# azedarach/matrix-factorization-case-studies

Hardware: AMD Instinct MI355X
Metric: AA SPG outer iterations/sec (synthetic 100000x4096, k=32) (higher is better)
Workload: dtype f32; 1 GPU; AA n=100000 p=4096 k=32, X row-sharded over 1 GPU(s), init=random, delta=0, dictionary spg max_iterations=1, default weights QP; parallelism=rows/1

## Files before the change

matrix-factorization-case-studies_amd/csrc/aa_internal.h:

```cpp
#pragma once
#include <hip/hip_runtime.h>

#include <cstdarg>
#include <cstdio>
#include <cstdlib>
#include <cstring>
#include <string>
#include <vector>

#include "../../include/aa_hip.h"

namespace aa {

void set_error(const char *fmt, ...);

#define AA_CHECK_HIP(expr)                                                              \
    do {                                                                                \
        hipError_t e__ = (expr);                                                        \
        if (e__ != hipSuccess) {                                                        \
            aa::set_error("%s:%d: %s -> %s", __FILE__, __LINE__, #expr,                 \
                          hipGetErrorString(e__));                                      \
            return AA_ERR_HIP;                                                          \
        }                                                                               \
    } while (0)
// ... 165 lines not shown
    hipStream_t stream = nullptr;
    hipStream_t stream2 = nullptr;
    hipStream_t stream3 = nullptr;
    hipEvent_t evFork = nullptr, evJoin = nullptr;
    DevBuf slotCosts, slotCounters, slotStates, slotCost0;
    int slots_R = 0, slots_k = 0, slots_stride = 0, slots_max_outer = 0;
    bool slots_aa = false, slots_started = false;
    unsigned slots_cold = 0;
    unsigned slots_cold_cols = 0xffffffffu;
    DevBuf slotSaveP, slotSaveGr;
    DevBuf slotSnapP;
    aa_iter_params slots_ip;
    aa_spg_params slots_sp, slots_scale_sp;
    aa_gpnh_params slots_gp;
    aa_qp_params slots_qp;
    DevBuf qpLive;
    long qp_live_cap = 0;
    int qp_live_epoch = 0;
    char pass_names[2][48] = {{0}, {0}};
    char qp_names[192] = {0};
    char spg_path[512] = {0};
    bool spg_path_full = false;
    bool qp_tail_pending = false;
    hipEvent_t evFork2 = nullptr, evJoin2 = nullptr;
    bool qp_perm_ready = false;
    long qp_perm_n = 0;
    bool side_pending = false;
    DevBuf tmpTall2, redPartial2, redOut2, proj2, projList2, projSegCnt2;
    int projPassHint2[4] = {0, 0, 0, 0};
    bool projWarm2[4] = {false, false, false, false};
    bool time_gemm = false;
    std::vector<hipEvent_t> gemmEvents[2];
    const int *qp_tail_rows = nullptr;
    const unsigned int *qp_tail_count = nullptr;
    Comm *comm = nullptr;
    P2P *p2p = nullptr;
    int rank = 0, world = 1;
    bool force_comm = false;
    struct RidePost {
        bool on = false;
        int kind = 0, mode = 0, NV = 0, slot = 0, gated = 0, stage_after = -1;
        unsigned max_mask = 0u;
        aa_spg_params sp;
        double *red = nullptr;
        ProjState *ps = nullptr;
        double *gather = nullptr;
        long count = 0;
    };
    RidePost ride, ride_grad;
    double *ride_dst = nullptr;
    long ride_count = 0;
    double *ride_gather_next = nullptr;
    bool weights_follow = false;
    bool ride_grad_next = false;

    int form = AA_FORM_DATA;
    long n = 0, n_pad = 0, p = 0, p_pad = 0, n_global = 0, row_offset = 0;
    DevBuf X;
    bool have_data = false;
    double trace = 0.0;
    bool have_trace = false;

    int k = 0, KP = 0;
    bool have_state = false, grams_valid = false, gpnh_valid = false;
    std::vector<double> alpha;
    std::vector<double> ZtZ, CKCt, CKZ;
    bool dict_inputs_overridden = false;

    DevBuf Ct, Zt, Dt, Gr, Gn, gk, gn, H, tmpTall;
    DevBuf P, Q, ZtX, Pw, Qw;
    DevBuf wideScratch;
    DevBuf partial;
    DevBuf groupFlags;
    DevBuf slabMode;
    DevBuf rlPartial;
    DevBuf redPartial;
    DevBuf gramOut;
    DevBuf gramState;
    DevBuf costDev;
    DevBuf costSlot;
    bool host_grams_valid = false;
    DevBuf redOut;
    DevBuf redGather;
    DevBuf listGather;
    DevBuf scalars;
    DevBuf proj;
    DevBuf projList, projSegCnt;
    DevBuf Mdev, alphaDev;
    DevBuf iterState, snapC, snapZ, snapAlpha;
    DevBuf qpIters;
    DevBuf qpPerm;
    DevBuf feat, featNorm;
    long feat_p = 0, feat_ld = 0;
    KernelSpec kernel;
    DevBuf crossX, crossNorm, crossV, rowNorm, xformCost;
    long cross_s = 0, cross_s_pad = 0;
    int cross_k = 0;
    KernelSpec cross;
    DevBuf scoreScratch;
    DevBuf fsScratch;
    int fs_k = 0;
    size_t fs_off_col = 0, fs_off_st = 0, fs_off_alive = 0;
    bool qp_iters_valid = false;
    bool linear_kernel = false;
    DevBuf qpStats;
    void *hostPinned = nullptr;
    size_t hostPinnedBytes = 0;

    long nslab = 0, rows_per_slab = 0;
    int tallBlocks = 0;
    int projPassHint[4] = {0, 0, 0, 0};
    bool projWarm[4] = {false, false, false, false};
    long projCounts[4] = {0, 0, 0, 0};
    bool projListShort[4] = {false, false, false, false};
    bool x_feasible = false;
    bool products_valid = false;
    bool ckz_valid = false;
};

void spg_name(Ctx *c, const char *fmt, ...) __attribute__((format(printf, 2, 3)));
#define SPG_NAME(...) spg_name(c, __VA_ARGS__)

inline bool has_stored_data(const Ctx *c) { return c->have_data && !c->kernel.kind && c->form == AA_FORM_DATA; }

int launch_reduce_rows(Ctx *c, const double *A_tall, double *out_wide, void *outT,
                       bool main_only = false, DevBuf *flag_buf = nullptr);
#define AA_SLAB_MODE_BYTES 256
#define REDUCE_SPARSE_DEFAULT_DEN(dtype) ((dtype) == AA_F32 ? 4 : 2)
int launch_reduce_rows_finish(Ctx *c, double *out_wide, void *outT, int extra_slabs);
int launch_reduce_rows_fixup(Ctx *c, const unsigned int *count_dev, const int *rows_dev,
                             const double *zslot, const double *Ztall);
int launch_row_local(Ctx *c, const void *B_wideT, double *out_tall);
int launch_stream_probe(Ctx *c, int variant);

int tall_setup(Ctx *c);
int launch_proj(Ctx *c, const double *x, const double *g, double a_const, int a_slot, int mode,
                const aa_spg_params *sp = nullptr, int stage_after = -1);
enum { PROJ_FEAS = 0, PROJ_ALPHA = 1, PROJ_DIR = 2, PROJ_RES = 3 };
int launch_grad(Ctx *c, const double *Graw, const double *H, double *gout, double scale,
                const double *d_for_dot , int dot_slot, double *xupd = nullptr,
                const aa_spg_params *sp = nullptr, int stage_after = -1,
                const aa_spg_params *setup_sp = nullptr , double setup_fnorm = 0.0);
int launch_tall_axpy_lambda(Ctx *c, double *x, const double *d);
int launch_group_flags(Ctx *c, const double *A_tall, unsigned char *flags, unsigned int *counters);
int launch_tall_dot_scaled(Ctx *c, const double *x, const double *H, const double *alpha_dev,
                           int slot);
int launch_gram_tall(Ctx *c, const double *A, const double *B, double *out_dev, bool local_only = false);
int launch_ride_post(Ctx *c, Ctx::RidePost *rp, const double *gather);
#define AA_WIDE_TAIL(KP) ((size_t)(KP) * (KP) + (size_t)64 * 4 * (KP))
int launch_gram_wide(Ctx *c, const double *A, const double *B, double *out_dev);
int launch_scale_gram(Ctx *c, double *dst, const double *src);
int launch_aa_cost(Ctx *c, double *out_dev, int *slot_counter_dev = nullptr, const LoopJudge *judge = nullptr);
int launch_set_scalars(Ctx *c, double trace, double fnorm);
int launch_wide_axpy_lambda(Ctx *c, double *P, const double *Q, void *PT);
int launch_wide_to_T(Ctx *c, const double *src, void *dstT);
int launch_transpose_wide_to_tall(Ctx *c, const double *wide, double *tall);
int launch_transpose_tall_to_wide(Ctx *c, const double *tall, double *wide, void *wideT);
int launch_scalar_stage(Ctx *c, int stage, const aa_spg_params *sp, int it);
int launch_linesearch_fused(Ctx *c, const aa_spg_params *sp, double *cost_out, int *cost_slot);
int launch_dict_setup(Ctx *c, const aa_spg_params *sp, double fnorm, unsigned slotmask = 0xffffffffu);
int launch_iter_judge(Ctx *c, const LoopJudge &jd, const double *costs, bool judged, bool wide_dict);
int launch_cost_carry(Ctx *c, double *costs, int *slot, double cost0);
int launch_scale_factors(Ctx *c, const aa_spg_params *sp, double delta_box, const LoopJudge &jd,
                         const double *costs, const int *slot);
int launch_col_has_nan(Ctx *c, const void *raw_dev, int host_dtype, long ld, long n_total, long p_full,
                       const double *w_dev , unsigned char *flags_dev);
int launch_gather_weight(Ctx *c, const void *raw_dev, int host_dtype, long ld, long row0, long n,
                         const int *idx_dev, long p_valid, const double *w_dev);
int launch_data_to_double(Ctx *c, double *out_dev);
#define AA_MOMENT_MAX_SLABS 2048
long moment_slab_rows(long n, long p_pad, long *nslab_out);
int launch_col_moments(Ctx *c, double *partial_dev , double *mean_dev ,
                       double *var_dev );
int launch_affine_rows(Ctx *c, const void *owner_X, long row0, const double *shift_dev ,
                       const double *scale_dev );
#define AA_MAX_COEF_ROWS 16
int launch_col_weighted_sums(Ctx *c, int G, const double *At_dev , const int *grp_dev ,
                             const double *centre_dev ,
                             double *partial_dev , double *out_dev );
int launch_model_rows(Ctx *c, const void *owner_X, long row0, const int *grp_dev, const double *shift_dev,
                      const double *icpt_dev, const double *slope_dev, const double *t_dev, const double *scale_dev,
                      void *dst = nullptr );
int launch_gather_rows(Ctx *c, const void *owner_X, int owner_dtype, long owner_ld, const long *idx_dev,
                       void *dst = nullptr );
int launch_features_from_data(Ctx *c, const void *owner_X, int owner_dtype, long owner_ld, long n, long p, double *F,
                              long ldf);
int launch_gpnh_solve(Ctx *c, double lambda, int *ok_dev);
int launch_gpnh_solve_slots(Ctx *c, double lambda);
int launch_gpnh_cost_slots(Ctx *c, double lambda, unsigned mask, int what, const JudgeRule &rule, bool form_gram);
int launch_gpnh_snap_slots(Ctx *c);
int launch_aa_cost_slots(Ctx *c, int what, const JudgeRule &rule);
int launch_aa_snap_slots(Ctx *c);
int launch_qp_slots_aa(Ctx *c, const aa_qp_params *p);
int launch_qp_slots(Ctx *c, int R, int k, const double *gram_dev, const aa_qp_params *p);
bool gpnh_cost_can_gram(const Ctx *c);
int launch_gpnh_cost(Ctx *c, double lambda, double *out_dev, int *slot_counter, bool from_wide = false,
                     bool gram_w = false, const LoopJudge *judge = nullptr);
enum { ST_INIT_F = 0, ST_ALPHA = 1, ST_LINESEARCH = 2, ST_BB = 3, ST_CONV = 4 };
int launch_row_sqnorm_sum(Ctx *c, double *trace_out_host);
int launch_distance_column(Ctx *c, long j_local, int owner_has_row, const double *xj_host, double *d_host);
int kernel_kv(Ctx *c, const double *V_tall, double *out_tall);
int kernel_cross(Ctx *c);
int launch_poly_trace(Ctx *c, double *trace_out_host);
int launch_row_norms(Ctx *c, const double *F, long ld, long p, long rows, double *nrm);
int launch_kernel_transform_cost(Ctx *c, const double *A_dev, const double *d_dev, double *part, double *out_host);
int launch_kernel_sample_residuals(Ctx *c, const double *A_dev, int kind, const double *d_dev, const double *nrm_dev,
                                   double *r_dev, double *dout_dev, double *part);
int launch_furthest_sum(Ctx *c, int k, int start, const int *exclude_host, int n_ex, int extra_steps,
                        int *selected_host, int *tie_host);
int fetch_furthest_sum_state(Ctx *c, double *sums, unsigned char *alive, double *column, int *cur, int *tie,
                             int *selected);
int launch_row_broadcast(Ctx *c, long j_local, bool own);
int launch_proj_side(Ctx *c, const double *x, const double *g, double a_const, int a_slot, int mode,
                     const aa_spg_params *sp, int stage_after);
int join_side(Ctx *c);
inline hipError_t ctx_memcpy(Ctx *c, void *dst, const void *src, size_t nbytes, hipMemcpyKind kind)
{
    if (join_side(c) != AA_OK) return hipErrorUnknown;
    hipError_t e = hipMemcpyAsync(dst, src, nbytes, kind, c->stream);
    if (e != hipSuccess) return e;
    return hipStreamSynchronize(c->stream);
}
inline hipError_t ctx_memcpy2d(Ctx *c, void *dst, size_t dpitch, const void *src, size_t spitch, size_t width,
                               size_t height, hipMemcpyKind kind)
{
    if (join_side(c) != AA_OK) return hipErrorUnknown;
    hipError_t e = hipMemcpy2DAsync(dst, dpitch, src, spitch, width, height, kind, c->stream);
    if (e != hipSuccess) return e;
    return hipStreamSynchronize(c->stream);
}
inline hipError_t ctx_memset(Ctx *c, void *dst, int value, size_t nbytes)
{
    return hipMemsetAsync(dst, value, nbytes, c->stream);
}
bool side_available(const Ctx *c);
int side_begin(Ctx *c);
int side_begin_behind(Ctx *c);
int side_end(Ctx *c);
extern int g_proj_res_side, g_grad_side;
int proj_poll_multirank(Ctx *c);
int launch_residual_cost(Ctx *c, const double *Ztall, const double *Wwide, const double *alpha_dev,
                         double *out_host );
int launch_residual_scores(Ctx *c, double *col_host, double *row_host, double *sse_host, bool fetch = true);

int launch_qp(Ctx *c, const double *A_host, const double *Btall, long stride_j, long stride_t,
              const double *bscale_host , double *Ztall, int ldz, long n, int k,
              const aa_qp_params *p, int *iters_dev, aa_qp_stats *stats,
              const double *gram_dev = nullptr, bool defer_tail = false);
#define QP_FIX_SLABS 32
int launch_qp_tail_fixup(Ctx *c, double *Ztall);
int launch_simplex_rows_generic(hipStream_t s, const double *in, double *out, long rows, long cols);

extern int g_use_graph;
extern int g_proj_mode, g_proj_small, g_proj_list_cap, g_proj_check_always;
extern int g_fuse_finalize, g_fin_in_last, g_gram_side, g_setup_in_grad;
extern int g_pack_comm, g_pq_mfma;
extern int g_row_local_variant, g_row_local_split, g_row_local_acc64, g_f64_mfma;
extern int g_reduce_sparse, g_reduce_sparse_max;
extern int g_qp_pass_cap, g_qp_mode, g_qp_quad_cap, g_qp_sort;
extern int g_qp_fused_order, g_qp_wave_lazy, g_qp_quad_lazy;
extern int g_qp_overlap_tail, g_qp_live;

int comm_unique_id(void *id128);
int comm_init(Ctx *c, const void *id128, int rank, int world);
void comm_destroy(Ctx *c);
int comm_allreduce(Ctx *c, double *dev, long count, int op);
int p2p_export(Ctx *c, int world, void *handle64);
int p2p_init(Ctx *c, const void *handles, int rank, int world);
int p2p_check(Ctx *c);

}
```

matrix-factorization-case-studies_amd/csrc/kernels_tall.hip:

```cpp
#include "aa_internal.h"

#include <utility>

namespace aa {

typedef double f64x4 __attribute__((ext_vector_type(4)));

__device__ __forceinline__ void store_agent(double *p, double v)
{
    __hip_atomic_store(reinterpret_cast<unsigned long long *>(p), (unsigned long long)__double_as_longlong(v),
                       __ATOMIC_RELAXED, __HIP_MEMORY_SCOPE_AGENT);
}
__device__ __forceinline__ double load_agent(const double *p)
{
    return __longlong_as_double((long long)__hip_atomic_load(reinterpret_cast<const unsigned long long *>(p),
                                                             __ATOMIC_RELAXED, __HIP_MEMORY_SCOPE_AGENT));
}

template <int KP, int NV, int NT = 256>
__device__ __forceinline__ void block_col_combine(const double (&v)[NV], unsigned max_mask,
                                                  double *sm, double *dst, bool agent = false)
{
    constexpr int RS = NT / KP;
    const int t = threadIdx.x, comp = t % KP, rsub = t / KP;
// ... 1026 lines not shown
            for (int ti = 0; ti < T; ++ti)
#pragma unroll
                for (int reg = 0; reg < 4; ++reg) {
                    const long row = ru + lr + 4 * reg;
                    const int comp = 16 * ti + lc;
                    if (row < n && comp < k) {
                        const long e = row * KP + o + comp;
                        dot += d[e] * g[e];
                    }
                }
        }
    }
    sm[threadIdx.x] = dot;
    __syncthreads();
    for (int q = 128; q > 0; q >>= 1) {
        if ((int)threadIdx.x < q) sm[threadIdx.x] += sm[threadIdx.x + q];
        __syncthreads();
    }
    double *dst = partial + (size_t)blockIdx.x * KP;
    if ((int)threadIdx.x < k) dst[o + threadIdx.x] = threadIdx.x == 0 ? sm[0] : 0.0;
    if (r == 0)
        for (int i = R * k + threadIdx.x; i < KP; i += 256) dst[i] = 0.0;
}

template <int KP>
__global__ __launch_bounds__(256) void k_tall_dot_scaled(const double *__restrict__ x,
                                                         const double *__restrict__ H,
                                                         const double *__restrict__ alpha, long n,
                                                         long rows_pb, int k,
                                                         double *__restrict__ partial)
{
    __shared__ double sm[256];
    constexpr int RS = 256 / KP;
    const int t = threadIdx.x, comp = t % KP, rsub = t / KP;
    const long rb = (long)blockIdx.x * rows_pb;
    long re = rb + rows_pb;
    if (re > n) re = n;
    double v[1] = {0.0};
    if (comp < k) {
        const double al = alpha ? alpha[comp] : 1.0;
        for (long r = rb + rsub; r < re; r += RS) v[0] += x[r * KP + comp] * H[r * KP + comp] * al;
    }
    block_col_combine<KP, 1>(v, 0u, sm, partial + (size_t)blockIdx.x * KP);
}

__global__ __launch_bounds__(256) void k_tall_axpy(double *__restrict__ x,
                                                   const double *__restrict__ d,
                                                   const double *__restrict__ scal, long elems)
{
    const long i = (long)blockIdx.x * 256 + threadIdx.x;
    if (i < elems) x[i] = x[i] + scal[SC_LAMBDA] * d[i];
}

template <typename T>
__global__ __launch_bounds__(256) void k_wide_axpy(double *__restrict__ P,
                                                   const double *__restrict__ Q,
                                                   const double *__restrict__ scal, long elems,
                                                   T *__restrict__ PT, long ld = 0, int kslot = 0, int R = 0)
{
    const long i = (long)blockIdx.x * 256 + threadIdx.x;
    if (i < elems) {
        if (kslot > 0) {
            const int r = (int)((i / ld) / kslot);
            scal += (size_t)(r < R ? r : 0) * AA_SC_STRIDE;
        }
        const double v = P[i] + scal[SC_LAMBDA] * Q[i];
        P[i] = v;
        if (PT) PT[i] = (T)v;
    }
}

template <typename T>
__global__ __launch_bounds__(256) void k_wide_to_T(const double *__restrict__ src, long elems,
                                                   T *__restrict__ dst)
{
    const long i = (long)blockIdx.x * 256 + threadIdx.x;
    if (i < elems) dst[i] = (T)src[i];
}

template <int KP>
__global__ __launch_bounds__(256) void k_gram_tall(const double *__restrict__ A,
                                                   const double *__restrict__ B, long n_pad,
                                                   long rows_pb, double *__restrict__ partial)
{
    constexpr int T = KP / 16;
    __shared__ double comb[3][KP * KP];
    const int wave = threadIdx.x >> 6, lane = threadIdx.x & 63;
    const int lr = lane >> 4, lc = lane & 15;
    const long rb = (long)blockIdx.x * rows_pb;
    long re = rb + rows_pb;
    if (re > n_pad) re = n_pad;
    f64x4 acc[T][T];
#pragma unroll
    for (int ti = 0; ti < T; ++ti)
#pragma unroll
        for (int tj = 0; tj < T; ++tj) acc[ti][tj] = (f64x4){0.0, 0.0, 0.0, 0.0};
    constexpr int UG = 4;
    for (long r = rb + 4 * wave; r < re; r += 16 * UG) {
        double av[UG][T], bv[UG][T];
#pragma unroll
        for (int u = 0; u < UG; ++u) {
            const long rr = r + 16 * u + lr;
#pragma unroll
            for (int ti = 0; ti < T; ++ti) {
                av[u][ti] = A[rr * KP + 16 * ti + lc];
                bv[u][ti] = B[rr * KP + 16 * ti + lc];
// ... 846 lines not shown
            return AA_OK;
        }
        long count = (long)c->world * NV * c->KP;
        if (c->ride_grad.on) count = region + (long)c->world * c->ride_grad.NV * c->KP;
        AA_CHECK(comm_allreduce(c, gather, count, 0));
        if (c->ride_grad.on) AA_CHECK(launch_ride_post(c, &c->ride_grad, gather + region));
        hipLaunchKernelGGL(k_post, dim3(1), dim3(256), 0, c->stream, kind, mode, red, c->KP, c->k, ps,
                           c->scalars.as<double>(), slot, gated ? 1 : 0, (const double *)gather,
                           c->world, NV, max_mask, stage_after, spv);
    }
    AA_CHECK_HIP(hipGetLastError());
    return AA_OK;
}

int launch_ride_post(Ctx *c, Ctx::RidePost *rp, const double *gather)
{
    rp->on = false;
    hipLaunchKernelGGL(k_post, dim3(1), dim3(256), 0, c->stream, rp->kind, rp->mode, rp->red, c->KP, c->k, rp->ps,
                       c->scalars.as<double>(), rp->slot, rp->gated, gather, c->world, rp->NV, rp->max_mask,
                       rp->stage_after, rp->sp);
    AA_CHECK_HIP(hipGetLastError());
    return AA_OK;
}

#define TALL_DISPATCH_NT(NTHREADS, KERNEL, ...)                                             \
    do {                                                                                    \
        if (c->KP == 32)                                                                    \
            hipLaunchKernelGGL(KERNEL<32>, dim3(c->tallBlocks), dim3(NTHREADS), 0,          \
                               c->stream, __VA_ARGS__);                                     \
        else                                                                                \
            hipLaunchKernelGGL(KERNEL<64>, dim3(c->tallBlocks), dim3(NTHREADS), 0,          \
                               c->stream, __VA_ARGS__);                                     \
    } while (0)

#define TALL_DISPATCH(KERNEL, ...)                                                          \
    do {                                                                                    \
        if (c->KP == 32)                                                                    \
            hipLaunchKernelGGL(KERNEL<32>, dim3(c->tallBlocks), dim3(256), 0, c->stream,    \
                               __VA_ARGS__);                                                \
        else                                                                                \
            hipLaunchKernelGGL(KERNEL<64>, dim3(c->tallBlocks), dim3(256), 0, c->stream,    \
                               __VA_ARGS__);                                                \
    } while (0)

static int g_proj_hard_cap = 200;

int g_proj_mode = 0;
int g_proj_check_always = 0;
int g_pq_mfma = 1;
int g_pack_comm = 1;
int g_setup_in_grad = 1;
int g_gram_side = 0;
int g_grad_side = 1;
int g_proj_res_side = 1;
int g_proj_small = 1;
int g_fuse_finalize = 1;
int g_fin_in_last = 1;
int g_proj_list_cap = 2048;

static int proj_iterative_passes(Ctx *c, const double *wsrc, int mode, long rpb, int first_batch)
{
    double *part = c->redPartial.as<double>();
    const double *scal = c->scalars.as<double>();
    ProjState *ps = c->proj.as<ProjState>();
    int batch = first_batch;
    int total = 0;
    int hdr[2] = {0, 0};
    while (true) {
        for (int it = 0; it < batch; ++it) {
            TALL_DISPATCH(k_proj_pass, wsrc, (const double *)nullptr, 0.0, scal, -1, c->n, rpb,
                          c->k, (const ProjState *)ps, part);
            AA_CHECK(finalize_and_post(c, 2, 0u, POST_MICHELOT, 0, 0, true));
        }
        total += batch;
        AA_CHECK_HIP(hipMemcpyAsync(hdr, &ps->done, sizeof(hdr), hipMemcpyDeviceToHost, c->stream));
        AA_CHECK_HIP(hipStreamSynchronize(c->stream));
        if (hdr[0] || total >= g_proj_hard_cap) break;
        batch = 3;
    }
    c->projPassHint[mode] = hdr[1];
    return AA_OK;
}

int proj_poll_multirank(Ctx *c)
{
    if (!(c->world > 1 || c->force_comm) || !c->proj.p) return AA_OK;
    AA_CHECK(p2p_check(c));
    ProjState *ps = c->proj.as<ProjState>();
    int h[5] = {0, 0, 0, 0, 0};
    AA_CHECK_HIP(hipMemcpyAsync(h, &ps->overflow_sticky, sizeof(h), hipMemcpyDeviceToHost, c->stream));
    AA_CHECK_HIP(hipStreamSynchronize(c->stream));
    AA_REQUIRE(h[0] == 0, AA_ERR_STATE,
               "multi-rank projection: a candidate list outgrew the gather buffer between two polls "
               "(set option proj_check=1 or proj_mode=1) [flag %d, longest lists %d %d %d %d]", h[0], h[1],
               h[2], h[3], h[4]);
    int cap = g_proj_list_cap;
    if (cap * c->world > PROJ_LDS_CAP) cap = PROJ_LDS_CAP / c->world;
    for (int m = 0; m < 4; ++m) c->projListShort[m] = c->projWarm[m] && h[1 + m] > 0 && h[1 + m] <= cap / 2;
    return AA_OK;
}

int launch_proj(Ctx *c, const double *x, const double *g, double a_const, int a_slot, int mode,
                const aa_spg_params *sp, int stage_after)
{
    const long rpb = tall_rows_pb(c);
    double *part = c->redPartial.as<double>();
// ... 193 lines not shown
        ds.Mout = c->Mdev.as<double>();
        ds.gram = c->gramOut.as<double>();
        ds.sc = c->scalars.as<double>();
        ds.sp = *setup_sp;
    }
    long gb = (c->n + 63) / 64;
    if (gb > 1024) gb = 1024;
    if (gb < 1) gb = 1;
    const long rpb = round_up((c->n + gb - 1) / gb, 64);
    const int nb = (int)((c->n + rpb - 1) / rpb);
    double *part = c->redPartial.as<double>();
    double *pdot = d_for_dot ? part : (double *)nullptr;
    const int kslot = c->slots_aa ? c->slots_k : 0;
    if (kslot && d_for_dot) pdot = c->tmpTall.as<double>();
    if (c->KP == 32) {
        SPG_NAME("k_grad<32>:nb=%d:rpb=%ld", nb, rpb);
        hipLaunchKernelGGL(k_grad<32>, dim3(nb + ds.on), dim3(256), 0, c->stream, Graw, H,
                           (const double *)c->Mdev.as<double>(), (const double *)c->alphaDev.as<double>(),
                           scale, c->n, rpb, c->k, gout, d_for_dot, pdot, xupd,
                           (const double *)c->scalars.as<double>(), kslot, c->slots_R, ds);
    } else {
        SPG_NAME("k_grad<64>:nb=%d:rpb=%ld", nb, rpb);
        hipLaunchKernelGGL(k_grad<64>, dim3(nb + ds.on), dim3(256), 0, c->stream, Graw, H,
                           (const double *)c->Mdev.as<double>(), (const double *)c->alphaDev.as<double>(),
                           scale, c->n, rpb, c->k, gout, d_for_dot, pdot, xupd,
                           (const double *)c->scalars.as<double>(), kslot, c->slots_R, ds);
    }
    if (kslot && d_for_dot) {
        const dim3 gd((unsigned)nb, (unsigned)c->slots_R);
        if (c->KP == 32)
            hipLaunchKernelGGL(k_grad_dot_slots<32>, gd, dim3(256), 0, c->stream, (const double *)gout, d_for_dot,
                               c->n, rpb, kslot, c->slots_R, part);
        else
            hipLaunchKernelGGL(k_grad_dot_slots<64>, gd, dim3(256), 0, c->stream, (const double *)gout, d_for_dot,
                               c->n, rpb, kslot, c->slots_R, part);
    }
    AA_CHECK_HIP(hipGetLastError());
    if (d_for_dot) {
        if (sp && stage_after >= 0 && !g_fuse_finalize) {
            AA_CHECK(finalize_and_post(c, 1, 0u, POST_SCALAR_SUM, 0, dot_slot, false, nb));
            AA_CHECK(launch_scalar_stage(c, stage_after, sp, 0));
        } else {
            AA_CHECK(finalize_and_post(c, 1, 0u, POST_SCALAR_SUM, 0, dot_slot, false, nb, sp, stage_after));
        }
    }
    return AA_OK;
}

int launch_tall_axpy_lambda(Ctx *c, double *x, const double *d)
{
    const long elems = c->n * c->KP;
    hipLaunchKernelGGL(k_tall_axpy, dim3((unsigned)((elems + 255) / 256)), dim3(256), 0, c->stream,
                       x, d, c->scalars.as<double>(), elems);
    AA_CHECK_HIP(hipGetLastError());
    return AA_OK;
}

int launch_tall_dot_scaled(Ctx *c, const double *x, const double *H, const double *alpha_dev, int slot)
{
    const long rpb = tall_rows_pb(c);
    double *part = c->redPartial.as<double>();
    TALL_DISPATCH(k_tall_dot_scaled, x, H, alpha_dev, c->n, rpb, c->k, part);
    AA_CHECK(finalize_and_post(c, 1, 0u, POST_SCALAR_SUM, 0, slot, false));
    return AA_OK;
}

int launch_gram_tall(Ctx *c, const double *A, const double *B, double *out_dev, bool local_only)
{
    const int want = 256;
    long rpb = round_up((c->n_pad + want - 1) / want, 64);
    const int nb = (int)((c->n_pad + rpb - 1) / rpb);
    double *part = c->redPartial.as<double>();
    const int elems = c->KP * c->KP;
    if (c->KP == 32)
        hipLaunchKernelGGL(k_gram_tall<32>, dim3(nb), dim3(256), 0, c->stream, A, B, c->n_pad, rpb, part);
    else
        hipLaunchKernelGGL(k_gram_tall<64>, dim3(nb), dim3(256), 0, c->stream, A, B, c->n_pad, rpb, part);
    hipLaunchKernelGGL(k_gram_finalize, dim3((elems + 63) / 64), dim3(256), 0, c->stream, part,
                       nb, elems, out_dev);
    AA_CHECK_HIP(hipGetLastError());
    if ((c->world > 1 || c->force_comm) && !local_only) AA_CHECK(comm_allreduce(c, out_dev, elems, 0));
    return AA_OK;
}

__global__ __launch_bounds__(256) void k_scale_gram(double *__restrict__ dst,
                                                    const double *__restrict__ src,
                                                    const double *__restrict__ alpha, int k, int KP, int kslot = 0)
{
    const int e = blockIdx.x * 256 + threadIdx.x;
    if (e >= KP * KP) return;
    const int i = e / KP, j = e % KP;
    dst[e] = (i < k && j < k && (kslot == 0 || i / kslot == j / kslot)) ? alpha[i] * src[e] * alpha[j] : 0.0;
}

__device__ __forceinline__ double aa_cost_body(const double *__restrict__ state, const double *__restrict__ alpha,
                                               int k, int KP, double trace, double n_global, double *sm )
{
    const double *ZtZ = state, *CKCt = state + KP * KP, *CKZ = state + 2 * KP * KP;
    const int t = threadIdx.x;
    double acc = 0.0;
    for (int e = t; e < k * k; e += 256) {
        const int i = e / k, j = e % k;
        acc += alpha[i] * ZtZ[i * KP + j] * alpha[j] * CKCt[j * KP + i];
    }
    if (t < k) acc -= 2.0 * (alpha[t] * CKZ[t * KP + t]);
    sm[t] = acc;
// ... 2020 lines not shown
```

matrix-factorization-case-studies_amd/csrc/solver.hip:

```cpp
#include "aa_internal.h"

#include <climits>
#include <functional>
#include <mutex>

namespace aa {

int g_outer_nosync = 0;
int g_use_graph = 0;

static thread_local std::string g_err;

void set_error(const char *fmt, ...)
{
    char buf[1024];
    va_list ap;
    va_start(ap, fmt);
    vsnprintf(buf, sizeof(buf), fmt, ap);
    va_end(ap);
    g_err = buf;
}

static inline size_t esize(const Ctx *c) { return c->dtype == AA_F32 ? 4 : 8; }

// ... 214 lines not shown
        AA_CHECK(join_side(c));
        AA_CHECK(launch_row_local(c, operandT(c, c->ZtX, c->Qw), c->H.as<double>()));
    } else {
        if (c->qp_tail_pending) AA_CHECK(launch_qp_tail_fixup(c, c->Zt.as<double>()));
        AA_CHECK(launch_gram_tall(c, c->Zt.as<double>(), c->Zt.as<double>(), dev_ZtZ(c)));
        if (c->kernel.kind) {
            AA_CHECK(kernel_kv(c, c->Zt.as<double>(), c->H.as<double>()));
        } else {
            AA_CHECK(launch_transpose_tall_to_wide(c, c->Zt.as<double>(), c->ZtX.as<double>(),
                                                   operandT(c, c->ZtX, c->Qw)));
            AA_CHECK(launch_row_local(c, operandT(c, c->ZtX, c->Qw), c->H.as<double>()));
        }
    }
    AA_CHECK(launch_gram_tall(c, c->Ct.as<double>(), c->H.as<double>(), dev_CKZ(c)));
    c->ckz_valid = true;
    c->host_grams_valid = false;
    c->dict_inputs_overridden = false;
    return AA_OK;
}

static int prepare(Ctx *c, double *cost)
{
    AA_REQUIRE(c->have_state, AA_ERR_STATE, "set_state must precede prepare");
    AA_CHECK(ensure_trace(c));
    AA_CHECK(upload_alpha(c));
    AA_CHECK(refresh_after_weights(c));
    AA_CHECK(refresh_after_dictionary(c, true));
    c->grams_valid = true;
    if (cost) AA_CHECK(device_cost(c, cost));
    return AA_OK;
}

static unsigned slots_all_mask(const Ctx *c) { return c->slots_R >= 32 ? 0xffffffffu : ((1u << c->slots_R) - 1u); }
static bool slots_mixed(const Ctx *c) { return c->slots_aa && c->slots_cold != 0 && c->slots_cold != slots_all_mask(c); }

static int slots_save_P(Ctx *c)
{
    const size_t wide = (size_t)c->KP * c->p_pad * sizeof(double);
    AA_CHECK(c->slotSaveP.alloc(wide));
    AA_CHECK_HIP(hipMemcpyAsync(c->slotSaveP.p, c->P.p, wide, hipMemcpyDeviceToDevice, c->stream));
    return AA_OK;
}
static int slots_restore_P_warm(Ctx *c)
{
    const int k = c->slots_k;
    for (int r = 0; r < c->slots_R; ++r) {
        if ((c->slots_cold >> r) & 1u) continue;
        const size_t off = (size_t)r * k * c->p_pad;
        AA_CHECK_HIP(hipMemcpyAsync(c->P.as<double>() + off, c->slotSaveP.as<double>() + off,
                                    (size_t)k * c->p_pad * sizeof(double), hipMemcpyDeviceToDevice, c->stream));
    }
    if (c->dtype == AA_F32) AA_CHECK(launch_wide_to_T(c, c->P.as<double>(), operandT(c, c->P, c->Pw)));
    return AA_OK;
}

static int dictionary_update(Ctx *c, const aa_spg_params *sp, aa_spg_stats *st, bool refresh,
                             double *cost_out = nullptr, int *cost_slot = nullptr,
                             bool *cost_recorded = nullptr)
{
    AA_REQUIRE(c->have_state && (c->grams_valid || c->dict_inputs_overridden), AA_ERR_STATE,
               "dictionary_update needs prepare() or set_dictionary_inputs() first");
    AA_REQUIRE(sp->max_iterations >= 1, AA_ERR_ARG, "spg max_iterations must be >= 1");
    AA_REQUIRE(sp->memory <= 16, AA_ERR_ARG,
               "spg memory = %d exceeds the HIP backend limit of 16", sp->memory);
    const int k = c->k, KP = c->KP;
    const bool data = c->form == AA_FORM_DATA;
    if (cost_recorded) *cost_recorded = false;
    AA_CHECK(join_side(c));

    double *x = c->Ct.as<double>();
    double *gram = c->gramOut.as<double>();
    const size_t GS = (size_t)KP * KP;
    const double gscale = (data && !c->linear_kernel) ? 1.0 / (double)c->n_global : 1.0 / (double)k;

    const bool warm = c->x_feasible && c->products_valid;
    const bool fused = data && g_fuse_finalize;
    const bool fast = fused && warm && c->grams_valid && c->ckz_valid && !c->dict_inputs_overridden;
    const bool setup_in_grad = fast && g_setup_in_grad && !c->slots_aa;
    c->spg_path[0] = 0;
    c->spg_path_full = false;
    if (setup_in_grad) SPG_NAME("fast:in_grad");
    else if (fast) SPG_NAME("fast:k_dict_setup");
    else if (warm) SPG_NAME("warm");
    else SPG_NAME("cold");
    if (fast) {
        if (!setup_in_grad) AA_CHECK(launch_dict_setup(c, sp, (double)k));
    } else {
        AA_CHECK(launch_scale_gram(c, c->Mdev.as<double>(), dev_ZtZ(c)));
        AA_CHECK(launch_set_scalars(c, c->trace, (double)k));
        if (!c->x_feasible) AA_CHECK(launch_proj(c, x, nullptr, 0.0, -1, PROJ_FEAS));
        if (!warm) {
            if (data) {
                const bool mixed = slots_mixed(c);
                if (mixed) AA_CHECK(slots_save_P(c));
                AA_CHECK(launch_reduce_rows(c, x, c->P.as<double>(), operandT(c, c->P, c->Pw)));
                if (mixed) AA_CHECK(slots_restore_P_warm(c));
                AA_CHECK(launch_gram_wide(c, c->P.as<double>(), c->P.as<double>(), gram));
            } else {
                if (c->kernel.kind) {
                    AA_CHECK(kernel_kv(c, x, c->Gr.as<double>()));
                } else {
                    AA_CHECK(launch_reduce_rows(c, x, c->wideScratch.as<double>(), nullptr));
                    AA_CHECK(launch_transpose_wide_to_tall(c, c->wideScratch.as<double>(), c->Gr.as<double>()));
                }
                AA_CHECK(launch_gram_tall(c, c->Gr.as<double>(), x, gram));
            }
        } else {
            AA_CHECK_HIP(hipMemcpyAsync(gram, dev_CKCt(c), GS * sizeof(double), hipMemcpyDeviceToDevice, c->stream));
        }
        AA_CHECK(launch_tall_dot_scaled(c, x, c->H.as<double>(), c->alphaDev.as<double>(), SC_S1));
        AA_CHECK(launch_scalar_stage(c, ST_INIT_F, sp, 0));
        if (slots_mixed(c)) AA_CHECK(launch_dict_setup(c, sp, (double)k, slots_all_mask(c) & ~c->slots_cold));
        if (data && !warm) AA_CHECK(launch_row_local(c, operandT(c, c->P, c->Pw), c->Gr.as<double>()));
    }
    c->products_valid = false;
    AA_CHECK(launch_grad(c, c->Gr.as<double>(), c->H.as<double>(), c->gk.as<double>(), gscale, nullptr, 0, nullptr,
                         nullptr, -1, setup_in_grad ? sp : nullptr, (double)k));

    std::vector<double> sc(SC_COUNT, 0.0);
    int n_iter = -1, flags = 0;
    bool grad_on_side = false;
    for (int it = 0; it < sp->max_iterations; ++it) {
        n_iter = it;
        if (it == 0 && sp->alpha0 < 0.0) {
            AA_CHECK(launch_proj(c, x, c->gk.as<double>(), 1.0, -1, PROJ_ALPHA, sp, ST_ALPHA));
        }
        const bool multi = c->world > 1 || c->force_comm;
        if (multi && g_pack_comm && data && !c->slots_aa) c->ride_gather_next = c->Q.as<double>() + (size_t)KP * c->p_pad;
        AA_CHECK(launch_proj(c, x, c->gk.as<double>(), 0.0, SC_ALPHA, PROJ_DIR));
        if (data) {
            AA_CHECK(launch_reduce_rows(c, c->Dt.as<double>(), c->Q.as<double>(), nullptr, false, &c->groupFlags));
            if (fused) {
                const bool rec = cost_out && sp->max_iterations == 1;
                AA_CHECK(launch_linesearch_fused(c, sp, rec ? cost_out : nullptr, rec ? cost_slot : nullptr));
                if (rec && cost_recorded) *cost_recorded = true;
            } else {
                AA_CHECK(launch_gram_wide(c, c->P.as<double>(), c->Q.as<double>(), gram + GS));
                AA_CHECK(launch_gram_wide(c, c->Q.as<double>(), c->Q.as<double>(), gram + 2 * GS));
                AA_CHECK(launch_scalar_stage(c, ST_LINESEARCH, sp, 1));
                SPG_NAME("k_gram_wide<%d>x2;k_scalar_stage", KP);
            }
        } else {
            if (c->kernel.kind) {
                AA_CHECK(kernel_kv(c, c->Dt.as<double>(), c->Gn.as<double>()));
            } else {
                AA_CHECK(launch_reduce_rows(c, c->Dt.as<double>(), c->wideScratch.as<double>(), nullptr, false,
                                            &c->groupFlags));
                AA_CHECK(launch_transpose_wide_to_tall(c, c->wideScratch.as<double>(), c->Gn.as<double>()));
            }
            AA_CHECK(launch_gram_tall(c, c->Gn.as<double>(), x, gram + GS));
            AA_CHECK(launch_gram_tall(c, c->Gn.as<double>(), c->Dt.as<double>(), gram + 2 * GS));
            AA_CHECK(launch_gram_tall(c, c->Gr.as<double>(), c->Dt.as<double>(), gram + 3 * GS));
            AA_CHECK(launch_scalar_stage(c, ST_LINESEARCH, sp, 0));
            SPG_NAME("k_gram_tall<%d>x3;k_scalar_stage", KP);
        }
        if (data) {
            AA_CHECK(launch_wide_axpy_lambda(c, c->P.as<double>(), c->Q.as<double>(), operandT(c, c->P, c->Pw)));
            AA_CHECK(launch_row_local(c, operandT(c, c->P, c->Pw), c->Gn.as<double>()));
            grad_on_side = g_grad_side && sp->max_iterations == 1 && !st && side_available(c);
            if (grad_on_side) AA_CHECK(side_begin(c));
            if (multi && g_pack_comm && !c->slots_aa && g_proj_mode == 0 && g_fuse_finalize) c->ride_grad_next = true;
            AA_CHECK(launch_grad(c, c->Gn.as<double>(), c->H.as<double>(), c->gn.as<double>(), gscale,
                                 c->Dt.as<double>(), SC_DGN, x, sp, ST_BB));
        } else {
            AA_CHECK(launch_tall_axpy_lambda(c, x, c->Dt.as<double>()));
            AA_CHECK(launch_tall_axpy_lambda(c, c->Gr.as<double>(), c->Gn.as<double>()));
            AA_CHECK(launch_grad(c, c->Gr.as<double>(), c->H.as<double>(), c->gn.as<double>(), gscale,
                                 c->Dt.as<double>(), SC_DGN, nullptr, sp, ST_BB));
        }
        if (multi && g_pack_comm && data && !c->slots_aa && c->weights_follow && sp->max_iterations == 1 && !st &&
            g_fuse_finalize)
            c->ride_gather_next = c->ZtX.as<double>() + (size_t)KP * c->p_pad + (size_t)KP * KP;
        if (grad_on_side) {
            const int rc = launch_proj(c, x, c->gn.as<double>(), 1.0, -1, PROJ_RES, sp, ST_CONV);
            AA_CHECK(side_end(c));
            AA_CHECK(rc);
        } else if (sp->max_iterations == 1 && !st && data)
            AA_CHECK(launch_proj_side(c, x, c->gn.as<double>(), 1.0, -1, PROJ_RES, sp, ST_CONV));
        else
            AA_CHECK(launch_proj(c, x, c->gn.as<double>(), 1.0, -1, PROJ_RES, sp, ST_CONV));
        if (data) std::swap(c->Gr, c->Gn);
        std::swap(c->gk, c->gn);
        if (st || it + 1 < sp->max_iterations) {
            AA_CHECK_HIP(hipMemcpyAsync(sc.data(), c->scalars.p, SC_COUNT * sizeof(double),
                                        hipMemcpyDeviceToHost, c->stream));
            AA_CHECK_HIP(hipStreamSynchronize(c->stream));
            AA_CHECK(proj_poll_multirank(c));
            flags = (int)sc[SC_FLAGS];
            if (flags & (AA_SPG_FLAG_CONVERGED | AA_SPG_FLAG_MAX_FEVAL)) break;
        }
    }
    if (n_iter == sp->max_iterations - 1 && !(flags & AA_SPG_FLAG_CONVERGED))
        flags |= AA_SPG_FLAG_MAX_ITER;
    if (st) {
        st->f = sc[SC_F_OLD];
        st->n_iter = n_iter;
        st->n_feval = (int)sc[SC_NFEVAL];
        st->flags = flags;
        st->res_norm = sqrt(sc[SC_RES2]);
    }
    c->x_feasible = true;
    if (refresh) AA_CHECK(refresh_after_dictionary(c, false, fused));
    return AA_OK;
}

static int weights_update(Ctx *c, const aa_qp_params *qp, aa_qp_stats *stats)
{
    AA_REQUIRE(c->have_state && c->grams_valid, AA_ERR_STATE, "weights_update needs prepare() first");
    const bool defer = g_qp_overlap_tail && c->form == AA_FORM_DATA;
    AA_CHECK(c->qpIters.alloc((size_t)c->n * sizeof(int)));
// ... 10 lines not shown
    AA_CHECK(refresh_after_weights(c));
    AA_CHECK(join_side(c));
    return AA_OK;
}

}

using namespace aa;

struct aa_ctx {
    Ctx c;
};

extern "C" {

const char *aa_last_error(void) { return g_err.c_str(); }
int aa_version(void) { return 100; }

struct AaOption {
    const char *name;
    int *target;
    int lo, hi;
    bool flag;
};
static const AaOption kOptions[] = {
    {"row_local_variant", &g_row_local_variant, -1, 9, false},
    {"row_local_acc64", &g_row_local_acc64, 0, 2, false},
    {"row_local_split", &g_row_local_split, 0, 1, true},
    {"f64_mfma", &g_f64_mfma, 0, 3, false},
    {"reduce_sparse", &g_reduce_sparse, 0, 1, true},
    {"reduce_sparse_max", &g_reduce_sparse_max, -1, INT_MAX, false},
    {"proj_mode", &g_proj_mode, 0, 1, false},
    {"proj_small", &g_proj_small, INT_MIN, INT_MAX, false},
    {"proj_list_cap", &g_proj_list_cap, 1, 2048, false},
    {"proj_check", &g_proj_check_always, 0, 1, true},
    {"proj_res_side", &g_proj_res_side, 0, 1, true},
    {"fuse_finalize", &g_fuse_finalize, 0, 1, true},
    {"use_graph", &g_use_graph, 0, 1, true},
    {"outer_nosync", &g_outer_nosync, 0, 1, true},
    {"pq_mfma", &g_pq_mfma, 0, 1, true},
    {"qp_mode", &g_qp_mode, 0, 4, false},
    {"qp_pass_cap", &g_qp_pass_cap, 1, INT_MAX, false},
    {"qp_quad_cap", &g_qp_quad_cap, 0, INT_MAX, false},
    {"qp_sort", &g_qp_sort, 0, 1, true},
    {"qp_live", &g_qp_live, 0, 1, true},
    {"qp_overlap_tail", &g_qp_overlap_tail, 0, 1, true},
    {"qp_fused_order", &g_qp_fused_order, 0, 1, true},
    {"qp_wave_lazy", &g_qp_wave_lazy, 0, 1, true},
    {"qp_quad_lazy", &g_qp_quad_lazy, 0, 1, true},
    {"fin_in_last", &g_fin_in_last, 0, 1, true},
    {"setup_in_grad", &g_setup_in_grad, 0, 1, true},
    {"gram_side", &g_gram_side, 0, 1, true},
    {"grad_side", &g_grad_side, 0, 1, true},
    {"pack_comm", &g_pack_comm, 0, 1, true},
};

int aa_set_option(const char *name, int value)
{
    AA_REQUIRE(name != nullptr, AA_ERR_ARG, "null option name");
    for (const AaOption &o : kOptions) {
        if (strcmp(name, o.name)) continue;
        AA_REQUIRE(o.flag || (value >= o.lo && value <= o.hi), AA_ERR_ARG, "%s must be in %d..%d", o.name, o.lo, o.hi);
        *o.target = o.flag ? (value != 0) : value;
        return AA_OK;
    }
    set_error("unknown option '%s'", name);
    return AA_ERR_ARG;
}

int aa_device_count(int *count)
{
    int n = 0;
    AA_CHECK_HIP(hipGetDeviceCount(&n));
    *count = n;
    return AA_OK;
}

int aa_ctx_create(aa_ctx **out, int device, int dtype)
{
    AA_REQUIRE(out != nullptr, AA_ERR_ARG, "null ctx pointer");
    AA_REQUIRE(dtype == AA_F32 || dtype == AA_F64, AA_ERR_ARG, "bad dtype %d", dtype);
    int n = 0;
    AA_CHECK_HIP(hipGetDeviceCount(&n));
    AA_REQUIRE(n > 0, AA_ERR_HIP, "no HIP device visible");
    AA_REQUIRE(device >= 0 && device < n, AA_ERR_ARG, "device %d out of range (0..%d)", device, n - 1);
    AA_CHECK_HIP(hipSetDevice(device));
    aa_ctx *h = new aa_ctx();
    h->c.device = device;
    h->c.dtype = dtype;
    hipError_t e = hipStreamCreateWithFlags(&h->c.stream, hipStreamNonBlocking);
    if (e == hipSuccess) {
        int lo = 0, hi = 0;
        (void)hipDeviceGetStreamPriorityRange(&lo, &hi);
        e = hipStreamCreateWithPriority(&h->c.stream2, hipStreamNonBlocking, hi);
        if (e == hipSuccess) e = hipStreamCreateWithPriority(&h->c.stream3, hipStreamNonBlocking, hi);
    }
    if (e == hipSuccess) e = hipEventCreateWithFlags(&h->c.evFork, hipEventDisableTiming);
    if (e == hipSuccess) e = hipEventCreateWithFlags(&h->c.evJoin, hipEventDisableTiming);
    if (e != hipSuccess) {
        set_error("hipStreamCreate: %s", hipGetErrorString(e));
        delete h;
        return AA_ERR_HIP;
    }
    *out = h;
    return AA_OK;
}
// ... 629 lines not shown
    if (CKCt) memcpy(CKCt, c->CKCt.data(), kk * sizeof(double));
    if (CKZ) memcpy(CKZ, c->CKZ.data(), kk * sizeof(double));
    if (trace) *trace = c->trace;
    return AA_OK;
}

int aa_set_dictionary_inputs(aa_ctx *h, const double *KZ, const double *ZtZ, double trace)
{
    AA_REQUIRE(h && KZ && ZtZ, AA_ERR_ARG, "null argument");
    Ctx *c = &h->c;
    AA_REQUIRE(c->have_state, AA_ERR_STATE, "set_state first");
    AA_CHECK_HIP(hipSetDevice(c->device));
    AA_CHECK(upload_tall(c, c->H, KZ, c->k, 1, c->n, c->k));
    {
        std::vector<double> pad((size_t)c->KP * c->KP, 0.0);
        for (int i = 0; i < c->k; ++i)
            for (int j = 0; j < c->k; ++j) pad[(size_t)i * c->KP + j] = ZtZ[(size_t)i * c->k + j];
        AA_CHECK_HIP(ctx_memcpy(c, dev_ZtZ(c), pad.data(), pad.size() * sizeof(double), hipMemcpyHostToDevice));
    }
    c->host_grams_valid = false;
    c->trace = trace;
    c->have_trace = true;
    c->dict_inputs_overridden = true;
    return AA_OK;
}

int aa_dictionary_update(aa_ctx *h, const aa_spg_params *params, aa_spg_stats *stats)
{
    AA_REQUIRE(h && params, AA_ERR_ARG, "null argument");
    AA_CHECK_HIP(hipSetDevice(h->c.device));
    return dictionary_update(&h->c, params, stats, true);
}

int aa_weights_update(aa_ctx *h, const aa_qp_params *params, aa_qp_stats *stats)
{
    AA_REQUIRE(h && params, AA_ERR_ARG, "null argument");
    AA_CHECK_HIP(hipSetDevice(h->c.device));
    return weights_update(&h->c, params, stats);
}

static int aa_enqueue_iteration(Ctx *c, const aa_spg_params *spg, const aa_qp_params *qp,
                                const aa_spg_params *scale_spg, double delta, bool upd_dict, bool upd_w,
                                double *cd, int *slot, const LoopJudge *jd)
{
    AA_REQUIRE(jd || (upd_dict && upd_w && !scale_spg), AA_ERR_ARG,
               "an AA iteration without a judge runs both updates and no scale-factor stage");
    if (scale_spg) {
        AA_CHECK(ensure_ckz(c));
        AA_CHECK(launch_scale_factors(c, scale_spg, delta, *jd, cd, slot));
    }
    if (upd_dict) {
        bool recorded = false;
        c->weights_follow = upd_w;
        const int rcd = dictionary_update(c, spg, nullptr, true, cd, slot, &recorded);
        c->weights_follow = false;
        AA_CHECK(rcd);
        if (cd && !recorded) {
            AA_CHECK(ensure_ckz(c));
            AA_CHECK(launch_aa_cost(c, cd, slot));
        }
    } else {
        AA_CHECK(launch_cost_carry(c, cd, slot, jd->cost0));
    }
    if (upd_w) {
        AA_CHECK(weights_update(c, qp, nullptr));
        if (cd) AA_CHECK(launch_aa_cost(c, cd, slot, jd));
        if (jd) AA_CHECK(launch_iter_judge(c, *jd, cd, true, false));
    } else {
        AA_CHECK(join_side(c));
        AA_CHECK(launch_cost_carry(c, cd, slot, jd->cost0));
        AA_CHECK(launch_iter_judge(c, *jd, cd, false, false));
    }
    return AA_OK;
}

int aa_outer_iterations(aa_ctx *h, int n_outer, const aa_spg_params *spg, const aa_qp_params *qp,
                        double *costs)
{
    AA_REQUIRE(h && spg && qp, AA_ERR_ARG, "null argument");
    Ctx *c = &h->c;
    AA_CHECK_HIP(hipSetDevice(c->device));
    AA_CHECK(c->costDev.alloc((size_t)(2 * n_outer + 64) * sizeof(double)));
    AA_CHECK(c->costSlot.alloc(64));
    int *slot = c->costSlot.as<int>();
    double *cd = c->costDev.as<double>();
    AA_CHECK_HIP(hipMemsetAsync(slot, 0, sizeof(int), c->stream));
    auto one_iteration = [&]() -> int {
        return aa_enqueue_iteration(c, spg, qp, nullptr, 0.0, true, true, costs ? cd : nullptr, slot, nullptr);
    };
    const bool graph = g_use_graph && c->world <= 1 && !c->force_comm && c->form == AA_FORM_DATA &&
                       spg->max_iterations == 1 && n_outer >= 8 && !g_qp_overlap_tail && !g_qp_live &&
                       !c->time_gemm;
    int i = 0;
    const int eager = graph ? 2 : n_outer;
    for (; i < eager; ++i) AA_CHECK(one_iteration());
    if (graph) {
        const int pairs = (n_outer - i) / 2;
        hipGraph_t g = nullptr;
        hipGraphExec_t ge = nullptr;
        AA_CHECK_HIP(hipStreamBeginCapture(c->stream, hipStreamCaptureModeThreadLocal));
        int rc = one_iteration();
        if (rc == AA_OK) rc = one_iteration();
        hipError_t e = hipStreamEndCapture(c->stream, &g);
        if (rc != AA_OK || e != hipSuccess || !g) {
            if (rc == AA_OK) set_error("hipStreamEndCapture: %s (set option use_graph=0)", hipGetErrorString(e));
            if (g) (void)hipGraphDestroy(g);
            return rc != AA_OK ? rc : AA_ERR_HIP;
        }
        e = hipGraphInstantiate(&ge, g, nullptr, nullptr, 0);
        for (int p = 0; p < pairs && e == hipSuccess; ++p) e = hipGraphLaunch(ge, c->stream);
        if (e == hipSuccess) e = hipStreamSynchronize(c->stream);
        if (ge) (void)hipGraphExecDestroy(ge);
        (void)hipGraphDestroy(g);
        if (e != hipSuccess) {
            set_error("hipGraph: %s (set option use_graph=0)", hipGetErrorString(e));
            return AA_ERR_HIP;
        }
        i += 2 * pairs;
        for (; i < n_outer; ++i) AA_CHECK(one_iteration());
    }
    if (g_outer_nosync && !costs) return AA_OK;
    if (costs && n_outer > 0)
        AA_CHECK_HIP(hipMemcpyAsync(costs, c->costDev.p, (size_t)2 * n_outer * sizeof(double),
                                    hipMemcpyDeviceToHost, c->stream));
    AA_CHECK_HIP(hipStreamSynchronize(c->stream));
    AA_CHECK(proj_poll_multirank(c));
    return AA_OK;
}

struct LoopRecords {
    double *cd;
    int *slot;
    IterState *st;
};

static int loop_records_begin(Ctx *c, int n_max, LoopRecords *rec)
{
    AA_CHECK(c->costDev.alloc((size_t)(2 * n_max + 64) * sizeof(double)));
    AA_CHECK(c->costSlot.alloc(64));
    AA_CHECK(c->iterState.alloc(sizeof(IterState)));
    rec->cd = c->costDev.as<double>();
    rec->slot = c->costSlot.as<int>();
    rec->st = c->iterState.as<IterState>();
    AA_CHECK_HIP(hipMemsetAsync(rec->slot, 0, sizeof(int), c->stream));
    AA_CHECK_HIP(hipMemsetAsync(rec->st, 0, sizeof(IterState), c->stream));
    return AA_OK;
}

static int run_device_loop(Ctx *c, const LoopRecords &rec, const aa_iter_params *ip, double cost0, double *costs,
                           aa_iter_stats *stats, bool poll_multirank, bool stop_not_definite,
                           const std::function<int(int)> &enqueue, const std::function<int()> &restore,
                           bool *restored = nullptr)
{
    const int n_max = ip->max_outer;
    if (restored) *restored = false;
    IterState hs;
    memset(&hs, 0, sizeof(hs));
    int done = 0;
    while (done < n_max) {
        const int batch = n_max - done < ip->check_every ? n_max - done : ip->check_every;
        for (int b = 0; b < batch; ++b) AA_CHECK(enqueue(done + b));
        done += batch;
        AA_CHECK_HIP(hipMemcpyAsync(&hs, rec.st, sizeof(hs), hipMemcpyDeviceToHost, c->stream));
        AA_CHECK_HIP(hipStreamSynchronize(c->stream));
        if (poll_multirank) AA_CHECK(proj_poll_multirank(c));
        if (hs.stop || (stop_not_definite && hs.not_definite)) break;
    }
    memset(stats, 0, sizeof(*stats));
    stats->reserved = done;
    if (stop_not_definite && hs.not_definite) {
        stats->error_stage = 3;
        stats->n_iter = -1;
        stats->cost = cost0;
        return AA_OK;
    }
    const int last = hs.stop ? hs.stop_iter : n_max - 1;
    AA_CHECK_HIP(ctx_memcpy(c, costs, rec.cd, (size_t)2 * (last + 1) * sizeof(double), hipMemcpyDeviceToHost));
    stats->n_iter = last;
    stats->converged = hs.converged;
    stats->error_stage = hs.error_stage;
    stats->error_iter = hs.error_stage ? hs.stop_iter : -1;
    stats->spg_flags = hs.spg_flags;
    stats->cost = costs[2 * last + 1];
    if (hs.stop && hs.stop_iter < done - 1 && !hs.error_stage) {
        AA_CHECK(restore());
        if (restored) *restored = true;
    }
    return AA_OK;
}

int aa_iterate(aa_ctx *h, const aa_iter_params *ip, const aa_spg_params *spg, const aa_qp_params *qp,
               const aa_spg_params *scale_spg, double cost0, double *costs, aa_iter_stats *stats)
{
    AA_REQUIRE(h && ip && spg && qp && costs && stats, AA_ERR_ARG, "null argument");
    AA_REQUIRE(ip->max_outer >= 1 && ip->check_every >= 1, AA_ERR_ARG, "bad iteration counts");
    AA_REQUIRE(ip->criterion == 0 || ip->criterion == 1, AA_ERR_ARG, "bad stopping criterion");
    Ctx *c = &h->c;
    AA_CHECK_HIP(hipSetDevice(c->device));
    AA_REQUIRE(c->have_state && c->grams_valid, AA_ERR_STATE, "aa_iterate needs aa_prepare first");
    const size_t tall_bytes = (size_t)c->n_pad * c->KP * sizeof(double);
    AA_CHECK(c->snapC.alloc(tall_bytes));
    AA_CHECK(c->snapZ.alloc(tall_bytes));
    AA_CHECK(c->snapAlpha.alloc(64 * sizeof(double)));
    LoopRecords rec;
    AA_CHECK(loop_records_begin(c, ip->max_outer, &rec));
    const bool scale = scale_spg != nullptr && ip->delta != 0.0;
    if (scale) AA_REQUIRE(scale_spg->memory <= 16, AA_ERR_ARG, "spg memory > 16 unsupported");
    auto enqueue = [&](int it) -> int {
        const LoopJudge jd = loop_judge(ip, it, cost0, rec.st, 1);
        return aa_enqueue_iteration(c, spg, qp, scale ? scale_spg : nullptr, ip->delta, ip->update_dictionary != 0,
                                    ip->update_weights != 0, rec.cd, rec.slot, &jd);
    };
    auto read_alpha = [&](const DevBuf &src) -> int {
        std::vector<double> a(c->KP, 1.0);
        AA_CHECK_HIP(ctx_memcpy(c, a.data(), src.p, (size_t)c->KP * sizeof(double), hipMemcpyDeviceToHost));
        for (int i = 0; i < c->k; ++i) c->alpha[i] = a[i];
        return AA_OK;
// ... 1213 lines not shown
```

Baseline: 643.0 it/s.

## Skip SPG tail work in single-iteration dictionary updates inside the outer loop

When the dictionary SPG runs a single iteration inside the judged outer loop, the step now applies the lambda axpy and row-local product, swaps the gradient buffers and exits early. This skips the gradient, projection and line-search tail that would otherwise run after the last accepted step. A flagged tall axpy updates only the row groups marked active, cutting memory traffic. The conditions depend on host-side copies of loop state such as the SPG flags. If those copies are stale, the skipped tail could change which statistics and costs are recorded.

```diff
diff --git a/matrix-factorization-case-studies_amd/csrc/aa_internal.h b/matrix-factorization-case-studies_amd/csrc/aa_internal.h
--- a/matrix-factorization-case-studies_amd/csrc/aa_internal.h
+++ b/matrix-factorization-case-studies_amd/csrc/aa_internal.h
@@ -241,6 +241,8 @@
     long ride_count = 0;
     double *ride_gather_next = nullptr;
     bool weights_follow = false;
+    bool loop_update = false, loop_judged = false;
+    int loop_spg_flags = 0;
     bool ride_grad_next = false;
 
     int form = AA_FORM_DATA;
@@ -331,6 +333,7 @@
                 const aa_spg_params *sp = nullptr, int stage_after = -1,
                 const aa_spg_params *setup_sp = nullptr , double setup_fnorm = 0.0);
 int launch_tall_axpy_lambda(Ctx *c, double *x, const double *d);
+int launch_tall_axpy_lambda_flagged(Ctx *c, double *x, const double *d, const unsigned char *flags);
 int launch_group_flags(Ctx *c, const double *A_tall, unsigned char *flags, unsigned int *counters);
 int launch_tall_dot_scaled(Ctx *c, const double *x, const double *H, const double *alpha_dev,
                            int slot);
@@ -426,7 +429,7 @@
 int side_begin(Ctx *c);
 int side_begin_behind(Ctx *c);
 int side_end(Ctx *c);
-extern int g_proj_res_side, g_grad_side;
+extern int g_proj_res_side, g_grad_side, g_spg_tail;
 int proj_poll_multirank(Ctx *c);
 int launch_residual_cost(Ctx *c, const double *Ztall, const double *Wwide, const double *alpha_dev,
                          double *out_host );
@@ -446,6 +449,10 @@
 extern int g_pack_comm, g_pq_mfma;
 extern int g_row_local_variant, g_row_local_split, g_row_local_acc64, g_f64_mfma;
 extern int g_reduce_sparse, g_reduce_sparse_max;
+inline bool reduce_rows_flags_operand(const Ctx *c)
+{
+    return g_reduce_sparse && !c->time_gemm && (c->dtype == AA_F32 || g_f64_mfma);
+}
 extern int g_qp_pass_cap, g_qp_mode, g_qp_quad_cap, g_qp_sort;
 extern int g_qp_fused_order, g_qp_wave_lazy, g_qp_quad_lazy;
 extern int g_qp_overlap_tail, g_qp_live;
diff --git a/matrix-factorization-case-studies_amd/csrc/kernels_tall.hip b/matrix-factorization-case-studies_amd/csrc/kernels_tall.hip
--- a/matrix-factorization-case-studies_amd/csrc/kernels_tall.hip
+++ b/matrix-factorization-case-studies_amd/csrc/kernels_tall.hip
@@ -1102,6 +1102,32 @@
     if (i < elems) x[i] = x[i] + scal[SC_LAMBDA] * d[i];
 }
 
+template <int KP>
+__global__ __launch_bounds__(256) void k_tall_axpy_flagged(double *__restrict__ x, const double *__restrict__ d,
+                                                           const double *__restrict__ scal,
+                                                           const unsigned char *__restrict__ flags, long ngroups,
+                                                           long elems)
+{
+    constexpr int L = KP / 32;
+    const int lane = threadIdx.x & 63;
+    const long g0 = ((long)blockIdx.x * 4 + (threadIdx.x >> 6)) * 8;
+    if (g0 >= ngroups) return;
+    const unsigned long long bytes = *reinterpret_cast<const unsigned long long *>(flags + g0);
+    if (bytes == 0ull) return;
+    const double lam = scal[SC_LAMBDA];
+    for (int u = 0; u < 8; ++u) {
+        if (((bytes >> (8 * u)) & 0xffull) == 0ull) continue;
+#pragma unroll
+        for (int l = 0; l < L; ++l) {
+            const long e = (g0 + u) * (4 * KP) + 2 * (l * 64 + lane);
+            if (e >= elems) continue;
+            const double x0 = x[e], x1 = x[e + 1], d0 = d[e], d1 = d[e + 1];
+            x[e] = x0 + lam * d0;
+            x[e + 1] = x1 + lam * d1;
+        }
+    }
+}
+
 template <typename T>
 __global__ __launch_bounds__(256) void k_wide_axpy(double *__restrict__ P,
                                                    const double *__restrict__ Q,
@@ -2054,6 +2080,7 @@
 int g_setup_in_grad = 1;
 int g_gram_side = 0;
 int g_grad_side = 1;
+int g_spg_tail = 0;
 int g_proj_res_side = 1;
 int g_proj_small = 1;
 int g_fuse_finalize = 1;
@@ -2353,6 +2380,20 @@
     const long elems = c->n * c->KP;
     hipLaunchKernelGGL(k_tall_axpy, dim3((unsigned)((elems + 255) / 256)), dim3(256), 0, c->stream,
                        x, d, c->scalars.as<double>(), elems);
+    AA_CHECK_HIP(hipGetLastError());
+    return AA_OK;
+}
+
+int launch_tall_axpy_lambda_flagged(Ctx *c, double *x, const double *d, const unsigned char *flags)
+{
+    const long ngroups = c->n_pad / 4;
+    const dim3 grid((unsigned)((ngroups + 31) / 32));
+    if (c->KP == 32)
+        hipLaunchKernelGGL(k_tall_axpy_flagged<32>, grid, dim3(256), 0, c->stream, x, d,
+                           (const double *)c->scalars.as<double>(), flags, ngroups, c->n * c->KP);
+    else
+        hipLaunchKernelGGL(k_tall_axpy_flagged<64>, grid, dim3(256), 0, c->stream, x, d,
+                           (const double *)c->scalars.as<double>(), flags, ngroups, c->n * c->KP);
     AA_CHECK_HIP(hipGetLastError());
     return AA_OK;
 }
diff --git a/matrix-factorization-case-studies_amd/csrc/solver.hip b/matrix-factorization-case-studies_amd/csrc/solver.hip
--- a/matrix-factorization-case-studies_amd/csrc/solver.hip
+++ b/matrix-factorization-case-studies_amd/csrc/solver.hip
@@ -290,6 +290,15 @@
     }
     if (c->dtype == AA_F32) AA_CHECK(launch_wide_to_T(c, c->P.as<double>(), operandT(c, c->P, c->Pw)));
     return AA_OK;
+}
+
+static bool spg_tail_needed(const Ctx *c, const aa_spg_params *sp, const aa_spg_stats *st)
+{
+    if (g_spg_tail || st || sp->max_iterations > 1) return true;
+    if (c->form != AA_FORM_DATA || c->slots_aa || c->world > 1 || c->force_comm) return true;
+    if (!c->loop_update || c->dict_inputs_overridden) return true;
+    if (c->loop_judged && (sp->max_feval < 202 || !(c->loop_spg_flags & AA_SPG_FLAG_MAX_ITER))) return true;
+    return false;
 }
 
 static int dictionary_update(Ctx *c, const aa_spg_params *sp, aa_spg_stats *st, bool refresh,
@@ -358,6 +367,7 @@
     std::vector<double> sc(SC_COUNT, 0.0);
     int n_iter = -1, flags = 0;
     bool grad_on_side = false;
+    const bool tail = spg_tail_needed(c, sp, st);
     for (int it = 0; it < sp->max_iterations; ++it) {
         n_iter = it;
         if (it == 0 && sp->alpha0 < 0.0) {
@@ -394,6 +404,18 @@
         }
         if (data) {
             AA_CHECK(launch_wide_axpy_lambda(c, c->P.as<double>(), c->Q.as<double>(), operandT(c, c->P, c->Pw)));
+            if (!tail) {
+                if (reduce_rows_flags_operand(c))
+                    AA_CHECK(launch_tall_axpy_lambda_flagged(c, x, c->Dt.as<double>(),
+                                                             c->groupFlags.as<unsigned char>()));
+                else
+                    AA_CHECK(launch_tall_axpy_lambda(c, x, c->Dt.as<double>()));
+                AA_CHECK(launch_row_local(c, operandT(c, c->P, c->Pw), c->Gn.as<double>()));
+                spg_name(c, "tail:skip");
+                std::swap(c->Gr, c->Gn);
+                std::swap(c->gk, c->gn);
+                break;
+            }
             AA_CHECK(launch_row_local(c, operandT(c, c->P, c->Pw), c->Gn.as<double>()));
             grad_on_side = g_grad_side && sp->max_iterations == 1 && !st && side_available(c);
             if (grad_on_side) AA_CHECK(side_begin(c));
@@ -510,6 +532,7 @@
     {"setup_in_grad", &g_setup_in_grad, 0, 1, true},
     {"gram_side", &g_gram_side, 0, 1, true},
     {"grad_side", &g_grad_side, 0, 1, true},
+    {"spg_tail", &g_spg_tail, 0, 1, true},
     {"pack_comm", &g_pack_comm, 0, 1, true},
 };
 
@@ -1245,7 +1268,10 @@
     if (upd_dict) {
         bool recorded = false;
         c->weights_follow = upd_w;
+        c->loop_update = true;
+        c->loop_judged = jd != nullptr;
         const int rcd = dictionary_update(c, spg, nullptr, true, cd, slot, &recorded);
+        c->loop_update = c->loop_judged = false;
         c->weights_follow = false;
         AA_CHECK(rcd);
         if (cd && !recorded) {
@@ -1337,6 +1363,7 @@
     rec->st = c->iterState.as<IterState>();
     AA_CHECK_HIP(hipMemsetAsync(rec->slot, 0, sizeof(int), c->stream));
     AA_CHECK_HIP(hipMemsetAsync(rec->st, 0, sizeof(IterState), c->stream));
+    c->loop_spg_flags = 0;
     return AA_OK;
 }
 
@@ -1356,6 +1383,7 @@
         done += batch;
         AA_CHECK_HIP(hipMemcpyAsync(&hs, rec.st, sizeof(hs), hipMemcpyDeviceToHost, c->stream));
         AA_CHECK_HIP(hipStreamSynchronize(c->stream));
+        c->loop_spg_flags = hs.spg_flags;
         if (poll_multirank) AA_CHECK(proj_poll_multirank(c));
         if (hs.stop || (stop_not_definite && hs.not_definite)) break;
     }
```

Result: faster. 687.4 it/s (median of 6 runs) (+6.9%).
